# OllieBoyne/FIND

Hardware: AMD Instinct MI355X
Metric: deformed vertices x rendered views / sec (fwd+bwd) (higher is better)
Workload: dtype f32; 1 GPU; train_3d.yaml network-stage step: 16 feet x 6890-vertex template per GPU, 10002-vertex GT scans, chamf(5000)+smooth+texture(1000) losses, backward, Adam(main_params) step; nothing rendered, views:=1; feet_per_gpu=16, template_verts=6890, parallelism=dp1

## Files before the change

### find_amd/_lib.py

```python
import ctypes
import os
from ctypes import POINTER, Structure, c_char_p, c_float, c_int, c_int16, c_int32, c_int64, c_void_p

_PKG = os.path.dirname(os.path.abspath(__file__))
LIB_PATH = os.path.join(_PKG, 'lib', 'libfind_hip.so')
MAX_LAYERS = 8
ABI_VERSION = 3

_lib = None


class MlpParams(Structure):
	_fields_ = [
		('width', c_int32), ('in_dim', c_int32), ('pe_size', c_int32), ('n_trunk', c_int32),
		('n_disp', c_int32), ('n_col', c_int32), ('lat_disp', c_int32), ('lat_col', c_int32),
		('B', c_void_p),
		('trunk_w', c_void_p * MAX_LAYERS), ('trunk_b', c_void_p * MAX_LAYERS),
		('disp_w', c_void_p * MAX_LAYERS), ('disp_b', c_void_p * MAX_LAYERS),
		('col_w', c_void_p * MAX_LAYERS), ('col_b', c_void_p * MAX_LAYERS),
		('avg_col', c_void_p),
		('precision', c_int32),
	]


# ... 57 lines not shown
	'find_normal_map_bwd': (c_int, [_P, _P, _P, _I, _I, _I, _I, c_int, _P, _P]),
	'find_normal_loss_ws_bytes': (c_int64, [_I]),
	'find_normal_loss_fwd': (c_int, [_P, _P, _P, _I, _P, _P, _I, _P]),
	'find_normal_loss_bwd': (c_int, [_P, _P, _P, _I, _P, _P, _P, _P]),
	'find_point_face_ws_bytes': (c_int64, [_I, _I]),
	'find_point_face_fwd': (c_int, [_P, _P, _P, _P, _I, _I, _I, _I, _I, _P, _P, _P, _P, _I, _P]),
	'find_point_face_bwd': (c_int, [_P, _P, _P, _I, _P, _P, _P, _I, _I, _I, _I, _P, _P, _P]),
	'find_depth_bwd': (c_int, [POINTER(RenderParams), _P, _P, _I, _P, _P, _I, _I, _I, _I, _P, _P, _P, _P]),
	'find_depth_loss_ws_bytes': (c_int64, [_I, _I]),
	'find_depth_loss_fwd': (c_int, [_P, _P, _P, _I, _I, c_int, c_float, c_float, _P, _P, _P, _I, _P]),
	'find_depth_loss_bwd': (c_int, [_P, _P, _P, _I, _I, c_int, c_float, c_float, _P, _P, _P, _P]),
	'find_uv_sample': (c_int, [_P, _I, _I, _I, _P, _I, _P, _I, _I, _P, _P, _I, _I, _P, _P]),
	'find_render_frags': (c_int, [POINTER(RenderParams), _I, _I, _I, _I, _P, _P, _P, _P]),
	'find_adam_step': (c_int, [_I, _P, _P, _P, _P, _P, c_float, c_float, c_float, c_float, c_float, _I, _P]),
	'find_adam_step_dev': (c_int, [_I, _P, _P, _P, _P, _P, c_float, c_float, c_float, c_float, c_float, _P, _P]),
	'find_sgd_step': (c_int, [_I, _P, _P, _P, _P, c_float, c_float, c_float, c_float, c_int, c_int, _P]),
	'find_register_fwd': (c_int, [_P, _I, _P, _P, _I, _I, _P, _P]),
	'find_register_bwd_ws_bytes': (c_int64, [_I, _I]),
	'find_register_bwd': (c_int, [_P, _I, _P, _P, _P, _I, _I, _P, _P, _P, _I, _P]),
	'find_pca_fwd': (c_int, [_P, _I, _I, _P, _I, _P, _P]),
	'find_pca_bwd_ws_bytes': (c_int64, [_I, _I, _I]),
	'find_pca_bwd': (c_int, [_P, _I, _I, _P, _I, _P, _P, _I, _P]),
	'find_sample_points_fwd': (c_int, [_P, _P, _I, _P, _P, _I, _I, _I, _I, _P, _P, _P, _P]),
	'find_sample_points_bwd': (c_int, [_P, _I, _P, _P, _P, _I, _I, _I, _I, _P, _P]),
	'find_face_areas': (c_int, [_P, _P, _I, _I, _I, _I, _P, _P]),
	'find_nn_fwd': (c_int, [_P, _P, _P, _P, _I, _I, _I, _P, _P, _P]),
	'find_nn_bwd': (c_int, [_P, _P, _P, _P, _P, _I, _I, _I, _P, _P, _P]),
	'find_sample_surface_ws_bytes': (c_int64, [_I, _I]),
	'find_sample_surface_fwd': (c_int, [_P, _P, _I, _P, _I, _I, _I, _I, _P, _P, _P, _P, _P, _P, _I, _P]),
	'find_sample_surface_again': (c_int, [_P, _P, _I, _P, _I, _I, _I, _I, _P, _P, _P, _P, _P, _P, _I, _P]),
	'find_chamfer_ws_bytes': (c_int64, [_I, _I, _I]),
	'find_chamfer_fwd': (c_int, [_P, _P, _P, _P, _I, _I, _I, _P, _P, _I, _P]),
	'find_chamfer_bwd': (c_int, [_P, _P, _P, _P, _I, _I, _I, _P, _P, _I, _P, _P, _P]),
	'find_masked_mse_fwd': (c_int, [_P, _P, _I, _P, _P]),
	'find_masked_mse_bwd': (c_int, [_P, _P, _I, _P, _P, _P]),
	'find_image_mse_ws_bytes': (c_int64, []),
	'find_image_mse_fwd': (c_int, [_P, _P, _P, _P, _I, _I, _P, _P, _I, _P]),
	'find_image_mse_bwd': (c_int, [_P, _P, _P, _P, _I, _I, _P, _P, _P, _P]),
	'find_image_metrics_ws_bytes': (c_int64, [_I, _I]),
	'find_image_metrics': (c_int, [_P, _P, _P, _P, _P, _P, _I, _I, _I, _P, _P, _I, _P]),
	'find_smooth_loss_fwd': (c_int, [_P, _P, _P, _P, _P, _P, _I, _I, _I, _I, c_float, c_float, _P, _P, _I, _P]),
	'find_smooth_loss_bwd': (c_int, [_P, _P, _P, _P, _P, _P, _I, _I, _I, _I, c_float, c_float, _P, _P, _I, _P, _P]),
	'find_smooth_ws_bytes': (c_int64, [_I, _I, _I]),
	'find_smooth_fwd': (c_int, [_P, _P, _P, _P, _P, _P, _I, _I, _I, _I, _P, _P, _P, _I, _P]),
	'find_smooth_bwd': (c_int, [_P, _P, _P, _P, _P, _P, _I, _I, _I, _I, _P, _P, _P, _I, _P, _P]),
	'find_render_ws_bytes': (c_int64, [POINTER(RenderParams), _I, _I, _I, _I]),
	'find_render_fwd': (c_int, [POINTER(RenderParams), _P, _P, _I, _P, _P, _P, _I, _I, _I, _I, _P, _P, _P, _P, _P, _I, _P]),
	'find_render_bwd': (c_int, [POINTER(RenderParams), _P, _P, _I, _P, _P, _P, _I, _I, _I, _I, _P, _P, _P, _P, _P, _P, _I, _P]),
	'find_render_flags': (c_int, [_P, _P, _P]),
	'find_render_features_ws_bytes': (c_int64, [POINTER(RenderParams), _I, _I, _I]),
	'find_render_features_fwd': (c_int, [POINTER(RenderParams), _P, _P, _I, _P, _P, _I, _I, _I, _I, _P, _I, _P, _P, _I, _P, _I, _P]),
	'find_render_features_bwd': (c_int, [POINTER(RenderParams), _P, _P, _I, _P, _P, _I, _I, _I, _I, _P, _I, _P, _P, _P, _P, _P, _I, _P, _I, _P]),
	'find_points_render': (c_int, [POINTER(PointsParams), _P, _P, _P, _P, _I, _I, _I, _P, _P, _P, _P, _P]),
	'find_frames_u8': (c_int, [_P, _I, _I, _I, _I, c_int, _P, _P]),
}


def lib():
	global _lib
	if _lib is not None:
		return _lib
	if not os.path.exists(LIB_PATH):
		raise RuntimeError(f'find_amd: HIP library not built: {LIB_PATH} is missing. Run `python -m find_amd.build` '
						   '(or __graft_entry__.build()). There is no CPU fallback.')
	import torch
	L = ctypes.CDLL(LIB_PATH)
# ... 95 lines not shown
```

### find_amd/csrc/common.h

```cpp
#pragma once
#include <hip/hip_runtime.h>
#include <stdarg.h>
#include <stdint.h>
#include <stdio.h>
#include <string.h>
#include <algorithm>

#include "find_hip.h"

namespace find {

void set_error(const char* fmt, ...);
extern int g_raster_ablate;

constexpr int MLP_SWITCHES = 16 | 32 | 128;
constexpr int RASTER_SWITCHES = 8 | 16 | 256 | 512 | 1024 | 2048 | 4096 | 8192 | 16384 | 32768;

inline int check_launch(const char* what) {
	hipError_t e = hipGetLastError();
	if (e != hipSuccess) {
		set_error("%s: %s", what, hipGetErrorString(e));
		return FIND_ELAUNCH;
	}
	return FIND_OK;
}

inline int64_t align_up(int64_t x, int64_t a) { return (x + a - 1) / a * a; }
inline int64_t cdiv(int64_t a, int64_t b) { return (a + b - 1) / b; }

struct Carver {
	char* base;
	int64_t off;
	explicit Carver(void* p) : base(reinterpret_cast<char*>(p)), off(0) {}
	template <typename T>
	T* take(int64_t n) {
		T* r = reinterpret_cast<T*>(base + off);
		off += align_up(n * (int64_t)sizeof(T), 256);
		return r;
	}
};

}

#define FIND_REQUIRE(cond, ...)            \
	do {                                   \
		if (!(cond)) {                     \
			find::set_error(__VA_ARGS__);  \
			return FIND_EINVAL;            \
		}                                  \
// ... 26 lines not shown
```

### find_amd/csrc/geom.hip

```cpp
#include "common.h"

namespace find {
namespace geom {

__device__ __forceinline__ float3 ld3(const float* p) { return make_float3(p[0], p[1], p[2]); }
__device__ __forceinline__ float3 sub3(float3 a, float3 b) { return make_float3(a.x - b.x, a.y - b.y, a.z - b.z); }
__device__ __forceinline__ float3 cross3(float3 a, float3 b) {
	return make_float3(a.y * b.z - a.z * b.y, a.z * b.x - a.x * b.z, a.x * b.y - a.y * b.x);
}
__device__ __forceinline__ float norm3(float3 a) { return sqrtf(a.x * a.x + a.y * a.y + a.z * a.z); }

__global__ void face_areas_kernel(const float* __restrict__ verts, const int32_t* __restrict__ faces, int64_t faces_mesh_stride,
								  int n_verts, int n_faces, float* __restrict__ areas) {
	const int m = blockIdx.y;
	const int f = blockIdx.x * blockDim.x + threadIdx.x;
	if (f >= n_faces) return;
	const int32_t* fp = faces + (int64_t)m * faces_mesh_stride + (int64_t)f * 3;
	const float* vp = verts + (int64_t)m * n_verts * 3;
	if (fp[0] < 0) {
		areas[(int64_t)m * n_faces + f] = 0.f;
		return;
	}
	const float3 a = ld3(vp + 3 * fp[0]), b = ld3(vp + 3 * fp[1]), c = ld3(vp + 3 * fp[2]);
	areas[(int64_t)m * n_faces + f] = 0.5f * norm3(cross3(sub3(b, a), sub3(c, a)));
// ... 479 lines not shown
		float total = 0.f;
		for (int i = 0; i < 2 * n_clouds; ++i) total += __builtin_nontemporal_load(partial + i);
		*loss = total / (float)max(n_clouds, 1);
	}
}

__global__ void chamfer_bwd_kernel(const float* __restrict__ x, const int32_t* __restrict__ x_len, int p1_max, const float* __restrict__ y,
								   const int32_t* __restrict__ y_len, int p2_max, const unsigned long long* __restrict__ kx,
								   const unsigned long long* __restrict__ ky, const float* __restrict__ g_loss, int n_clouds,
								   float* __restrict__ d_x, float* __restrict__ d_y) {
	const int n = blockIdx.y, dir = blockIdx.z;
	const int i = blockIdx.x * blockDim.x + threadIdx.x;
	const int pa_max = dir ? p2_max : p1_max, pb_max = dir ? p1_max : p2_max;
	const int32_t* la = dir ? y_len : x_len;
	const int pa = la ? la[n] : pa_max;
	if (i >= pa) return;
	const unsigned long long v = (dir ? ky : kx)[(int64_t)n * pa_max + i];
	if (v == ~0ull) return;
	const int j = (int)(unsigned)v;
	const float* ap = (dir ? y : x) + ((int64_t)n * pa_max + i) * 3;
	const float* bp = (dir ? x : y) + ((int64_t)n * pb_max + j) * 3;
	const float g = 2.0f * (*g_loss) / ((float)n_clouds * (float)max(pa, 1));
	const float gx = g * (ap[0] - bp[0]), gy = g * (ap[1] - bp[1]), gz = g * (ap[2] - bp[2]);
	float* da = dir ? d_y : d_x;
	float* db = dir ? d_x : d_y;
	if (da) {
		float* o = da + ((int64_t)n * pa_max + i) * 3;
		unsafeAtomicAdd(o + 0, gx); unsafeAtomicAdd(o + 1, gy); unsafeAtomicAdd(o + 2, gz);
	}
	if (db) {
		float* o = db + ((int64_t)n * pb_max + j) * 3;
		unsafeAtomicAdd(o + 0, -gx); unsafeAtomicAdd(o + 1, -gy); unsafeAtomicAdd(o + 2, -gz);
	}
}

__global__ void nn_bwd_kernel(const float* __restrict__ x, const int32_t* __restrict__ x_len, const float* __restrict__ y,
							  const int32_t* __restrict__ idx, const float* __restrict__ w, int p1_max, int p2_max,
							  float* __restrict__ d_x, float* __restrict__ d_y) {
	const int n = blockIdx.y;
	const int i = blockIdx.x * blockDim.x + threadIdx.x;
	const int p1 = x_len ? x_len[n] : p1_max;
	if (i >= p1) return;
	const int64_t o = (int64_t)n * p1_max + i;
	const int j = idx[o];
	if (j < 0) return;
	const float g = 2.0f * w[o];
	const float* xp = x + o * 3;
	const float* yp = y + ((int64_t)n * p2_max + j) * 3;
	const float gx = g * (xp[0] - yp[0]), gy = g * (xp[1] - yp[1]), gz = g * (xp[2] - yp[2]);
	if (d_x) {
		d_x[o * 3 + 0] += gx; d_x[o * 3 + 1] += gy; d_x[o * 3 + 2] += gz;
	}
	if (d_y) {
		float* dy = d_y + ((int64_t)n * p2_max + j) * 3;
		atomicAdd(dy + 0, -gx); atomicAdd(dy + 1, -gy); atomicAdd(dy + 2, -gz);
	}
}

__global__ void cot_weights_kernel(const float* __restrict__ verts, const int32_t* __restrict__ faces, int n_verts, int n_faces,
								   float* __restrict__ fw) {
#pragma clang fp contract(off)
	const int m = blockIdx.y;
	const int f = blockIdx.x * blockDim.x + threadIdx.x;
	if (f >= n_faces) return;
	const int32_t* fp = faces + (int64_t)f * 3;
	const float* vp = verts + (int64_t)m * n_verts * 3;
// ... 823 lines not shown
	a.d[0] = NnDir{x, x_len, y, y_len, (int)p1_max, (int)p2_max, nullptr, nullptr, w.kx};
	a.d[1] = NnDir{y, y_len, x, x_len, (int)p2_max, (int)p1_max, nullptr, nullptr, w.ky};
	a.n_dirs = 2;
	a.counter = w.counter;
	const int64_t p_max = std::max(p1_max, p2_max);
	int np;
	nn_shape(cdiv(p_max, 128) * n * 2, std::min(p1_max, p2_max), &np, &a.splits);
	if (a.splits > 1) {
		hipError_t e = hipMemsetAsync(ws, 0xff, (size_t)w.key_bytes, s);
		if (e != hipSuccess) { set_error("find_chamfer_fwd: hipMemsetAsync: %s", hipGetErrorString(e)); return FIND_ELAUNCH; }
	}
	int rc = launch_nn(a, np, p_max, n, s);
	if (rc != FIND_OK) return rc;
	hipLaunchKernelGGL(chamfer_reduce_kernel, dim3((unsigned)n, 2), dim3(1024), 0, s, w.kx, x_len, (int)p1_max, w.ky, y_len, (int)p2_max, (int)n, w.partial, w.counter,
					   loss);
	FIND_LAUNCH_CHECK("chamfer_reduce_kernel");
	return FIND_OK;
}

extern "C" int find_chamfer_bwd(const float* x, const int32_t* x_len, const float* y, const int32_t* y_len, int64_t n, int64_t p1_max, int64_t p2_max,
								const float* g_loss, const void* ws, int64_t ws_bytes, float* d_x, float* d_y, void* stream) {
	FIND_REQUIRE(x && y && g_loss && ws, "find_chamfer_bwd: NULL argument");
	FIND_REQUIRE(d_x || d_y, "find_chamfer_bwd: both gradient outputs NULL");
	FIND_REQUIRE(!bad_dims(n, p1_max) && !bad_dims(n, p2_max), "find_chamfer_bwd: bad sizes");
	ChamferWs w;
	carve_chamfer(n, p1_max, p2_max, const_cast<void*>(ws), &w);
	if (ws_bytes < w.bytes) { set_error("find_chamfer_bwd: workspace too small"); return FIND_EWORKSPACE; }
	hipLaunchKernelGGL(chamfer_bwd_kernel, dim3((unsigned)cdiv(std::max(p1_max, p2_max), 256), (unsigned)n, 2), dim3(256), 0, (hipStream_t)stream, x, x_len,
					   (int)p1_max, y, y_len, (int)p2_max, w.kx, w.ky, g_loss, (int)n, d_x, d_y);
	FIND_LAUNCH_CHECK("chamfer_bwd_kernel");
	return FIND_OK;
}

extern "C" int64_t find_sample_surface_ws_bytes(int64_t n_meshes, int64_t n_faces) {
	if (bad_dims(n_meshes, n_faces)) return -1;
	return align_up(n_meshes * n_faces * (int64_t)sizeof(float), 256);
}

extern "C" int find_sample_surface_fwd(const float* verts, const int32_t* faces, int64_t faces_batch, const float* rnd, int64_t n_meshes, int64_t n_verts,
									   int64_t n_faces, int64_t n_samples, int32_t* face_idx, float* uv, float* out, const float* attr, float* attr_out,
									   void* ws, int64_t ws_bytes, void* stream) {
	FIND_REQUIRE(verts && faces && rnd && face_idx && uv && out && ws, "find_sample_surface_fwd: NULL argument");
	FIND_REQUIRE((attr == nullptr) == (attr_out == nullptr), "find_sample_surface_fwd: attr and attr_out must both be given or both NULL");
	FIND_REQUIRE(!bad_dims(n_meshes, n_samples) && !bad_dims(n_meshes, n_faces) && n_verts >= 1, "find_sample_surface_fwd: bad sizes");
	FIND_REQUIRE(faces_batch == 1 || faces_batch == n_meshes, "find_sample_surface_fwd: faces_batch must be 1 or n_meshes");
	if (ws_bytes < find_sample_surface_ws_bytes(n_meshes, n_faces)) { set_error("find_sample_surface_fwd: workspace too small"); return FIND_EWORKSPACE; }
	hipStream_t s = (hipStream_t)stream;
	const int64_t fstride = faces_batch == 1 ? 0 : n_faces * 3;
	hipLaunchKernelGGL(face_areas_kernel, dim3((unsigned)cdiv(n_faces, 256), (unsigned)n_meshes), dim3(256), 0, s, verts, faces, fstride, (int)n_verts, (int)n_faces,
					   (float*)ws);
	hipLaunchKernelGGL(area_scan_kernel, dim3((unsigned)n_meshes), dim3(1024), 0, s, (int)n_faces, (float*)ws);
	hipLaunchKernelGGL(sample_surface_kernel, dim3((unsigned)cdiv(n_samples, 256), (unsigned)n_meshes), dim3(256), 0, s, verts, faces, fstride, (const float*)ws, rnd,
					   (int)n_verts, (int)n_faces, (int)n_samples, face_idx, uv, out, attr, attr_out);
	FIND_LAUNCH_CHECK("sample_surface");
	return FIND_OK;
}

extern "C" int find_sample_surface_again(const float* verts, const int32_t* faces, int64_t faces_batch, const float* rnd, int64_t n_meshes, int64_t n_verts,
										 int64_t n_faces, int64_t n_samples, int32_t* face_idx, float* uv, float* out, const float* attr, float* attr_out,
										 const void* ws, int64_t ws_bytes, void* stream) {
	FIND_REQUIRE(verts && faces && rnd && face_idx && uv && out && ws, "find_sample_surface_again: NULL argument");
	FIND_REQUIRE((attr == nullptr) == (attr_out == nullptr), "find_sample_surface_again: attr and attr_out must both be given or both NULL");
	FIND_REQUIRE(!bad_dims(n_meshes, n_samples) && !bad_dims(n_meshes, n_faces) && n_verts >= 1, "find_sample_surface_again: bad sizes");
	FIND_REQUIRE(faces_batch == 1 || faces_batch == n_meshes, "find_sample_surface_again: faces_batch must be 1 or n_meshes");
	if (ws_bytes < find_sample_surface_ws_bytes(n_meshes, n_faces)) { set_error("find_sample_surface_again: workspace too small"); return FIND_EWORKSPACE; }
	const int64_t fstride = faces_batch == 1 ? 0 : n_faces * 3;
// ... 131 lines not shown
```

### find_amd/functional.py

```python
import ctypes

import torch

from . import _lib
from ._lib import MlpGrads, MlpParams, check, current_stream, ptr


def _require_gpu(*tensors):
	for t in tensors:
		if t is None:
			continue
		if not t.is_cuda:
			raise RuntimeError('find_amd: the HIP path needs tensors on a ROCm device (got a CPU tensor); '
							   'there is no CPU fallback -- use oracle/ only for testing')
		if t.dtype != torch.float32 and t.is_floating_point():
			raise RuntimeError(f'find_amd: fp32 tensors required, got {t.dtype}')


def _c(t):
	return None if t is None else t.contiguous()


def _ws(nbytes, device):
	return torch.empty(max(int(nbytes), 256), dtype=torch.uint8, device=device)
# ... 613 lines not shown
		F = faces.shape[-2]
		out = torch.empty(N, S, 3, device=verts.device, dtype=torch.float32)
		aout = torch.empty_like(out) if attr is not None else None
		check(L.find_sample_points_fwd(ptr(verts), ptr(faces), fb, ptr(face_idx), ptr(uv), N, V, F, S, ptr(out), ptr(attr), ptr(aout),
									   current_stream(verts.device)), 'find_sample_points_fwd')
		ctx.save_for_backward(faces, face_idx, uv)
		ctx.dims = (N, V, F, S, fb)
		ctx.has_attr = attr is not None
		ctx.set_materialize_grads(False)
		if attr is None:
			return out
		return out, aout

	@staticmethod
	def backward(ctx, g_out, g_attr=None):
		L = _lib.lib()
		faces, face_idx, uv = ctx.saved_tensors
		N, V, F, S, fb = ctx.dims

		def scatter(g):
			if g is None:
				return None
			d = torch.zeros(N, V, 3, device=g.device, dtype=torch.float32)
			check(L.find_sample_points_bwd(ptr(faces), fb, ptr(face_idx), ptr(uv), ptr(_c(g)), N, V, F, S, ptr(d), current_stream(g.device)),
				  'find_sample_points_bwd')
			return d

		d_verts = scatter(g_out) if ctx.needs_input_grad[0] else None
		d_attr = scatter(g_attr) if (ctx.has_attr and ctx.needs_input_grad[4]) else None
		return d_verts, None, None, None, d_attr


def sample_points(verts, faces, face_idx, uv, attr=None):
	return _SamplePoints.apply(verts, faces, face_idx, uv, attr)


class _NoCtx:
	needs_input_grad = (False,) * 64

	def save_for_backward(self, *tensors):
		pass

	def mark_non_differentiable(self, *tensors):
		pass

	def set_materialize_grads(self, value):
		pass


_NO_CTX = _NoCtx()
CACHE_AREA_SUMS = _os.environ.get('FIND_CACHE_AREA_SUMS', '1') != '0'
_AREA_SUMS = {}
_AREA_SUM_OWNERS = {}


class _SampleSurface(torch.autograd.Function):

	@staticmethod
	def forward(ctx, verts, faces, rnd, attr):
		_require_gpu(verts, rnd, attr)
		L = _lib.lib()
		verts_in, faces_in = verts, faces
		verts, rnd, attr = _c(verts), _c(rnd), _c(attr)
		faces = _faces_i32(faces)
		N, V, _ = verts.shape
		S = rnd.shape[1]
		if rnd.shape != (N, S, 3):
# ... 32 lines not shown
					del _AREA_SUM_OWNERS[k]
		ctx.save_for_backward(faces, face_idx, uv)
		ctx.dims = (N, V, F, S, fb)
		ctx.has_attr = attr is not None
		ctx.mark_non_differentiable(face_idx, uv)
		ctx.set_materialize_grads(False)
		if attr is None:
			return out, face_idx, uv
		return out, aout, face_idx, uv

	@staticmethod
	def backward(ctx, g_out, *rest):
		L = _lib.lib()
		faces, face_idx, uv = ctx.saved_tensors
		N, V, F, S, fb = ctx.dims
		g_attr = rest[0] if ctx.has_attr else None

		def scatter(g):
			if g is None:
				return None
			d = torch.zeros(N, V, 3, device=g.device, dtype=torch.float32)
			check(L.find_sample_points_bwd(ptr(faces), fb, ptr(face_idx), ptr(uv), ptr(_c(g)), N, V, F, S, ptr(d), current_stream(g.device)),
				  'find_sample_points_bwd')
			return d

		d_verts = scatter(g_out) if ctx.needs_input_grad[0] else None
		d_attr = scatter(g_attr) if (ctx.has_attr and ctx.needs_input_grad[3]) else None
		return d_verts, None, None, d_attr


def sample_surface(verts, faces, rnd, attr=None):
	if torch.is_grad_enabled() and (verts.requires_grad or (attr is not None and attr.requires_grad)):
		r = _SampleSurface.apply(verts, faces, rnd, attr)
	else:
		r = _SampleSurface.forward(_NO_CTX, verts, faces, rnd, attr)
	if attr is None:
		return r[0], None, r[1], r[2]
	return r


class _PointFace(torch.autograd.Function):

	@staticmethod
	def forward(ctx, points, verts, faces, p_len):
		_require_gpu(points, verts)
		L = _lib.lib()
		points, verts = _c(points), _c(verts)
		faces = _faces_i32(faces)
		if points.dim() != 3 or verts.dim() != 3 or points.shape[-1] != 3 or verts.shape[-1] != 3 or verts.shape[0] != points.shape[0]:
			raise RuntimeError(f'find_amd.point_face_distance: points (N, P, 3) and verts (N, V, 3) expected, got {tuple(points.shape)} / {tuple(verts.shape)}')
		N, P, _ = points.shape
		V = verts.shape[1]
		if faces.dim() not in (2, 3) or faces.shape[-1] != 3 or (faces.dim() == 3 and faces.shape[0] not in (1, N)):
			raise RuntimeError(f'find_amd.point_face_distance: faces (F, 3) or ({N}, F, 3) expected, got {tuple(faces.shape)}')
		fb = 1 if faces.dim() == 2 else faces.shape[0]
		F = faces.shape[-2]
		dev = points.device
		pl = None if p_len is None else torch.as_tensor(p_len).to(device=dev, dtype=torch.int32).contiguous()
		dist2 = torch.empty(N, P, device=dev, dtype=torch.float32)
		idx = torch.empty(N, P, device=dev, dtype=torch.int32)
		bary = torch.empty(N, P, 3, device=dev, dtype=torch.float32)
		ws = _ws(L.find_point_face_ws_bytes(N, P), dev)
		check(L.find_point_face_fwd(ptr(points), ptr(pl), ptr(verts), ptr(faces), fb, N, P, V, F, ptr(dist2), ptr(idx), ptr(bary), ptr(ws), ws.numel(),
									current_stream(dev)), 'find_point_face_fwd')
		ctx.save_for_backward(points, verts, faces, idx, bary)
		ctx.dims = (N, P, V, F, fb)
# ... 70 lines not shown
		P2 = y.shape[1]
		if y.shape[0] != N:
			raise RuntimeError('find_amd.chamfer_distance: batch mismatch')
		dev = x.device
		xl = None if x_len is None else x_len.to(device=dev, dtype=torch.int32).contiguous()
		yl = None if y_len is None else y_len.to(device=dev, dtype=torch.int32).contiguous()
		ws = _ws(L.find_chamfer_ws_bytes(N, P1, P2), dev)
		loss = torch.empty((), device=dev, dtype=torch.float32)
		check(L.find_chamfer_fwd(ptr(x), ptr(xl), ptr(y), ptr(yl), N, P1, P2, ptr(loss), ptr(ws), ws.numel(), current_stream(dev)), 'find_chamfer_fwd')
		ctx.save_for_backward(x, y, ws)
		ctx.lens = (xl, yl)
		return loss

	@staticmethod
	def backward(ctx, g):
		L = _lib.lib()
		x, y, ws = ctx.saved_tensors
		xl, yl = ctx.lens
		N, P1, _ = x.shape
		P2 = y.shape[1]
		need_x, need_y = ctx.needs_input_grad[0], ctx.needs_input_grad[1]
		if not (need_x or need_y):
			return None, None, None, None
		buf = torch.zeros((N * P1 * 3 if need_x else 0) + (N * P2 * 3 if need_y else 0), device=x.device, dtype=torch.float32)
		d_x = buf[:N * P1 * 3].view(N, P1, 3) if need_x else None
		d_y = buf[buf.numel() - N * P2 * 3:].view(N, P2, 3) if need_y else None
		check(L.find_chamfer_bwd(ptr(x), ptr(xl), ptr(y), ptr(yl), N, P1, P2, ptr(_c(g)), ptr(ws), ws.numel(), ptr(d_x), ptr(d_y), current_stream(x.device)),
			  'find_chamfer_bwd')
		return d_x, d_y, None, None


def chamfer_distance(x, y, x_lengths=None, y_lengths=None):
	return _Chamfer.apply(x, y, x_lengths, y_lengths), None


class _MaskedMSE(torch.autograd.Function):
	@staticmethod
	def forward(ctx, pred, target):
		_require_gpu(pred, target)
		L = _lib.lib()
		pred, target = _c(pred), _c(target.detach())
		if pred.shape != target.shape or pred.shape[-1] != 3:
			raise RuntimeError(f'find_amd.masked_mse: pred {tuple(pred.shape)} and target {tuple(target.shape)} must both be (..., 3)')
		loss = torch.empty((), device=pred.device, dtype=torch.float32)
		check(L.find_masked_mse_fwd(ptr(pred), ptr(target), pred.numel() // 3, ptr(loss), current_stream(pred.device)), 'find_masked_mse_fwd')
		ctx.save_for_backward(pred, target)
		return loss

	@staticmethod
	def backward(ctx, g):
		L = _lib.lib()
		pred, target = ctx.saved_tensors
		d = torch.empty_like(pred)
		check(L.find_masked_mse_bwd(ptr(pred), ptr(target), pred.numel() // 3, ptr(_c(g)), ptr(d), current_stream(pred.device)), 'find_masked_mse_bwd')
		return d, None


def masked_mse(pred, target):
	return _MaskedMSE.apply(pred, target)


class _ImageMSE(torch.autograd.Function):

	@staticmethod
	def forward(ctx, a, am, b, bm):
		_require_gpu(a, am, b, bm)
# ... 439 lines not shown
```

### find_amd/losses.py

```python
import itertools

import numpy as np
import torch

from . import functional as FN
from . import functional_render as FR
from .structures import Meshes, TexturesUV, TexturesVertex

nn = torch.nn


def sample_points_from_meshes(meshes: Meshes, num_samples: int = 10000, return_textures: bool = False, generator=None, draws=None):
	verts = meshes.verts_padded()
	faces = meshes.faces_shared()
	if faces is None:
		faces = meshes.faces_padded()
	N = verts.shape[0]
	tex = meshes.textures if return_textures else None
	if return_textures and not isinstance(tex, (TexturesUV, TexturesVertex)):
		raise NotImplementedError('return_textures needs TexturesVertex or TexturesUV')
	attr = tex.verts_features_padded()[..., :3].contiguous() if isinstance(tex, TexturesVertex) else None
	if draws is None:
		rnd = torch.rand(N, num_samples, 3, device=verts.device, generator=generator)
		pts, cols, face_idx, uv = FN.sample_surface(verts, faces, rnd, attr)
	else:
		face_idx, uv = draws
		r = FN.sample_points(verts, faces, face_idx, uv, attr)
		pts, cols = r if attr is not None else (r, None)
	if not return_textures:
		return pts
	if isinstance(tex, TexturesUV):
		su = uv[..., 0].sqrt()
		bary = torch.stack([1.0 - su, su * (1.0 - uv[..., 1]), su * uv[..., 1]], dim=-1)
		return pts, FR.uv_sample(tex.maps_padded(), tex.verts_uvs_padded(), tex.faces_uvs_padded(), face_idx, bary)
	return pts, cols


def _compact_by_mask(points, keep):
	order = torch.argsort((~keep).to(torch.int8), dim=1, stable=True)
	return torch.gather(points, 1, order.unsqueeze(-1).expand(-1, -1, 3)), keep.sum(dim=1).to(torch.int32)


def chamfer_distance(x, y, x_lengths=None, y_lengths=None):
	return FN.chamfer_distance(x, y, x_lengths, y_lengths)


def _mesh_faces(meshes):
	faces = meshes.faces_shared()
	return faces if faces is not None else meshes.faces_padded()


def point_mesh_distance(points, meshes: Meshes, lengths=None):
	return FN.point_face_distance(points, meshes.verts_padded(), _mesh_faces(meshes), lengths)


class TextureLossGTSpace(nn.Module):
	def forward(self, model, batch: dict, num_samples=1000, shapevec=None, texvec=None, posevec=None, gt_samples=None) -> torch.Tensor:
		mesh_gt = batch['mesh']
		sampled_verts, sampled_gt_colours = gt_samples if gt_samples is not None else sample_points_from_meshes(mesh_gt, num_samples=num_samples, return_textures=True)
		texvec = texvec if texvec is not None else batch.get('texvec', None)
		shapevec = shapevec if shapevec is not None else batch.get('shapevec', None)
		posevec = posevec if posevec is not None else batch.get('posevec', None)
		only_col = dict(want=('col',), defer_wgrad_join=True) if 'want' in getattr(getattr(model.forward, '__code__', None), 'co_varnames', ()) else {}
		res = model(sampled_verts.detach(), texvec=texvec, shapevec=shapevec, posevec=posevec, **only_col)
		return FN.masked_mse(res['col'], sampled_gt_colours)


class DisplacementLoss(nn.Module):
	def forward(self, model, res, batch, epoch, num_samples=5000, z_cutoff=None, gt_z_cutoff=None, gt_samples=None):
		if gt_samples is None:
			gt_samples = sample_points_from_meshes(batch['mesh'], num_samples=num_samples)
		pred_samples = sample_points_from_meshes(res['meshes'], num_samples=num_samples)
		if z_cutoff is not None:
			p, pl = _compact_by_mask(pred_samples, pred_samples[..., 2] <= z_cutoff)
			g, gl = _compact_by_mask(gt_samples, gt_samples[..., 2] <= z_cutoff)
			chamf_loss, _ = chamfer_distance(p, g, pl, gl)
		elif gt_z_cutoff is not None:
			g, gl = _compact_by_mask(gt_samples, gt_samples[..., 2] <= gt_z_cutoff)
			chamf_loss, _ = chamfer_distance(pred_samples, g, None, gl)
		else:
			chamf_loss, _ = chamfer_distance(pred_samples, gt_samples)
		return dict(loss=chamf_loss)


class MeshSmoothnessLoss(nn.Module):
	def forward(self, meshes: Meshes):
		faces = meshes.faces_shared()
		if faces is None:
			raise NotImplementedError('MeshSmoothnessLoss expects meshes sharing one topology (the template), as on the FIND path')
		verts = meshes.verts_padded()
		topo = FN.MeshTopology.get(faces, verts.shape[1])
		return FN.mesh_smoothness_loss(verts, topo, w_edge=10.0, w_lap=0.1)


class SilhouetteLoss(nn.Module):
	def forward(self, pred, gt):
		return FN.image_mse(pred, gt)


def draw_pairs(N, npairs=10):
	max_pairs = (N * (N - 1)) // 2
	npairs = min(npairs, max_pairs)
	all_pairs = list(itertools.permutations(np.arange(N), 2))
	np.random.shuffle(all_pairs)
	return np.array(all_pairs[:npairs], dtype=np.int32).reshape(-1, 2)
# ... 92 lines not shown
```

### include/find_hip.h

```cpp
#ifndef FIND_HIP_H
#define FIND_HIP_H

#include <stdint.h>

#ifdef __cplusplus
extern "C" {
#endif

#define FIND_ABI_VERSION 3

#define FIND_OK 0
#define FIND_EINVAL (-1)
#define FIND_EWORKSPACE (-2)
#define FIND_ELAUNCH (-3)

#define FIND_MAX_LAYERS 8

int find_abi_version(void);
const char* find_last_error(void);
const char* find_build_arch(void);

typedef struct find_ctx find_ctx;
int find_ctx_create(int device, find_ctx** out);
int find_ctx_destroy(find_ctx* ctx);
// ... 104 lines not shown
					  const float* d_out, int64_t n_feet, int64_t n_pts, float* d_disp, float* d_reg,
					  void* ws, int64_t ws_bytes, void* stream);

int find_pca_fwd(const float* coefs, int64_t V, int64_t B, const float* shapevec, int64_t n_feet, float* offsets, void* stream);
int64_t find_pca_bwd_ws_bytes(int64_t n_feet, int64_t V, int64_t B);
int find_pca_bwd(const float* coefs, int64_t V, int64_t B, const float* d_offsets, int64_t n_feet, float* d_shapevec, void* ws, int64_t ws_bytes,
				 void* stream);

int find_sample_points_fwd(const float* verts, const int32_t* faces, int64_t faces_batch, const int32_t* face_idx,
						   const float* uv, int64_t n_meshes, int64_t n_verts, int64_t n_faces, int64_t n_samples,
						   float* out, const float* attr, float* attr_out, void* stream);
int find_sample_points_bwd(const int32_t* faces, int64_t faces_batch, const int32_t* face_idx, const float* uv,
						   const float* d_out, int64_t n_meshes, int64_t n_verts, int64_t n_faces, int64_t n_samples,
						   float* d_verts, void* stream);
int find_face_areas(const float* verts, const int32_t* faces, int64_t faces_batch, int64_t n_meshes, int64_t n_verts,
					int64_t n_faces, float* areas, void* stream);
int64_t find_sample_surface_ws_bytes(int64_t n_meshes, int64_t n_faces);
int find_sample_surface_fwd(const float* verts, const int32_t* faces, int64_t faces_batch, const float* rnd, int64_t n_meshes,
							int64_t n_verts, int64_t n_faces, int64_t n_samples, int32_t* face_idx, float* uv, float* out,
							const float* attr, float* attr_out, void* ws, int64_t ws_bytes, void* stream);
int find_sample_surface_again(const float* verts, const int32_t* faces, int64_t faces_batch, const float* rnd, int64_t n_meshes,
							  int64_t n_verts, int64_t n_faces, int64_t n_samples, int32_t* face_idx, float* uv, float* out,
							  const float* attr, float* attr_out, const void* ws, int64_t ws_bytes, void* stream);

int find_nn_fwd(const float* x, const int32_t* x_len, const float* y, const int32_t* y_len, int64_t n,
				int64_t p1_max, int64_t p2_max, float* dist, int32_t* idx, void* stream);
int find_nn_bwd(const float* x, const int32_t* x_len, const float* y, const int32_t* idx, const float* w, int64_t n,
				int64_t p1_max, int64_t p2_max, float* d_x, float* d_y, void* stream);
int64_t find_chamfer_ws_bytes(int64_t n, int64_t p1_max, int64_t p2_max);
int find_chamfer_fwd(const float* x, const int32_t* x_len, const float* y, const int32_t* y_len, int64_t n, int64_t p1_max,
					 int64_t p2_max, float* loss, void* ws, int64_t ws_bytes, void* stream);
int find_chamfer_bwd(const float* x, const int32_t* x_len, const float* y, const int32_t* y_len, int64_t n, int64_t p1_max,
					 int64_t p2_max, const float* g_loss, const void* ws, int64_t ws_bytes, float* d_x, float* d_y, void* stream);

int find_masked_mse_fwd(const float* pred, const float* target, int64_t n_pts, float* loss, void* stream);
int find_masked_mse_bwd(const float* pred, const float* target, int64_t n_pts, const float* g_loss, float* d_pred, void* stream);
int64_t find_image_mse_ws_bytes(void);
int find_image_mse_fwd(const float* a, const float* a_mask, const float* b, const float* b_mask, int64_t n_pix, int64_t channels, float* loss,
					   void* ws, int64_t ws_bytes, void* stream);
int find_image_mse_bwd(const float* a, const float* a_mask, const float* b, const float* b_mask, int64_t n_pix, int64_t channels,
					   const float* g_loss, float* d_a, float* d_a_mask, void* stream);

#define FIND_IMAGE_METRIC_SQ 0
#define FIND_IMAGE_METRIC_SQ_EACH 1
#define FIND_IMAGE_METRIC_SQ_COMMON 2
#define FIND_IMAGE_METRIC_INTER 3
#define FIND_IMAGE_METRIC_UNION 4
#define FIND_IMAGE_METRIC_WSQ 5
#define FIND_IMAGE_METRIC_W 6
#define FIND_IMAGE_METRIC_COUNT 7
int64_t find_image_metrics_ws_bytes(int64_t n_img, int64_t n_pix);
int find_image_metrics(const float* pred, const float* gt, const float* pred_mask, const float* gt_mask, const uint8_t* hide, const float* weight,
					   int64_t n_img, int64_t n_pix, int64_t channels, double* sums, void* ws, int64_t ws_bytes, void* stream);

int64_t find_smooth_ws_bytes(int64_t n_meshes, int64_t n_verts, int64_t n_faces);
int find_smooth_fwd(const float* verts, const int32_t* faces, const int32_t* vf_off, const int32_t* vf_items,
					const int32_t* nbr_off, const int32_t* nbr_idx, int64_t n_meshes, int64_t n_verts, int64_t n_faces,
					int64_t n_edges, float* loss_edge, float* loss_lap, void* ws, int64_t ws_bytes, void* stream);
int find_smooth_bwd(const float* verts, const int32_t* faces, const int32_t* vf_off, const int32_t* vf_items,
					const int32_t* nbr_off, const int32_t* nbr_idx, int64_t n_meshes, int64_t n_verts, int64_t n_faces,
					int64_t n_edges, const float* g_edge, const float* g_lap, void* ws, int64_t ws_bytes, float* d_verts,
					void* stream);
int find_smooth_loss_fwd(const float* verts, const int32_t* faces, const int32_t* vf_off, const int32_t* vf_items,
						 const int32_t* nbr_off, const int32_t* nbr_idx, int64_t n_meshes, int64_t n_verts, int64_t n_faces,
						 int64_t n_edges, float w_edge, float w_lap, float* loss, void* ws, int64_t ws_bytes, void* stream);
int find_smooth_loss_bwd(const float* verts, const int32_t* faces, const int32_t* vf_off, const int32_t* vf_items,
// ... 81 lines not shown
```

Measured before the change: 73.17 million vertices*views/s.

## Fuse chamfer backward with surface-sample scatter into vertex gradients in LDS

Adds a fused backward kernel that computes chamfer gradients for the sampled points and scatters them through barycentric weights straight into a per-workgroup LDS image of vertex gradients. It replaces the separate chamfer backward, the sample-points backward and their global atomics. Large batches are split into slices whose partial results go to a workspace and are summed by a second kernel. The Python loss path uses it by default when the shapes fit in LDS, which adds LDS CAS loops and a dependence on sample metadata attached to tensors.

Result: faster. 74.97 million vertices*views/s, median of 6 (+2.5%).

```diff
diff --git a/find_amd/_lib.py b/find_amd/_lib.py
--- a/find_amd/_lib.py
+++ b/find_amd/_lib.py
@@ -113,6 +113,8 @@
 	'find_chamfer_ws_bytes': (c_int64, [_I, _I, _I]),
 	'find_chamfer_fwd': (c_int, [_P, _P, _P, _P, _I, _I, _I, _P, _P, _I, _P]),
 	'find_chamfer_bwd': (c_int, [_P, _P, _P, _P, _I, _I, _I, _P, _P, _I, _P, _P, _P]),
+	'find_chamfer_surface_bwd_ws_bytes': (c_int64, [_I, _I, _I]),
+	'find_chamfer_surface_bwd': (c_int, [_P, _P, _P, _I, _I, _I, _P, _P, _I, _P, _I, _P, _P, _I, _I, _P, _P, _I, _P]),
 	'find_masked_mse_fwd': (c_int, [_P, _P, _I, _P, _P]),
 	'find_masked_mse_bwd': (c_int, [_P, _P, _I, _P, _P, _P]),
 	'find_image_mse_ws_bytes': (c_int64, []),
diff --git a/find_amd/csrc/common.h b/find_amd/csrc/common.h
--- a/find_amd/csrc/common.h
+++ b/find_amd/csrc/common.h
@@ -14,7 +14,7 @@
 extern int g_raster_ablate;
 
 constexpr int MLP_SWITCHES = 16 | 32 | 128;
-constexpr int RASTER_SWITCHES = 8 | 16 | 256 | 512 | 1024 | 2048 | 4096 | 8192 | 16384 | 32768;
+constexpr int RASTER_SWITCHES = 8 | 16 | 256 | 512 | 1024 | 2048 | 4096 | 8192 | 16384 | 32768 | 0x70000;
 
 inline int check_launch(const char* what) {
 	hipError_t e = hipGetLastError();
diff --git a/find_amd/csrc/geom.hip b/find_amd/csrc/geom.hip
--- a/find_amd/csrc/geom.hip
+++ b/find_amd/csrc/geom.hip
@@ -535,6 +535,197 @@
 		float* o = db + ((int64_t)n * pb_max + j) * 3;
 		unsafeAtomicAdd(o + 0, -gx); unsafeAtomicAdd(o + 1, -gy); unsafeAtomicAdd(o + 2, -gz);
 	}
+}
+
+constexpr int SCB_THREADS = 1024, SCB_BATCH = 5;
+constexpr int64_t SCB_LDS_MAX = 160 * 1024;
+struct SurfBwdArgs {
+	const float *x, *y;
+	const int32_t* y_len;
+	const unsigned long long *kx, *ky;
+	const float* g_loss;
+	const int32_t* faces;
+	int64_t faces_mesh_stride;
+	const int32_t* face_idx;
+	const float* uv;
+	int p1, p2_max, n_clouds, n_verts, n_faces;
+	int range;
+	float* out;
+	int64_t out_foot_stride, out_slice_stride;
+};
+
+template <int N>
+__device__ __forceinline__ void lds_add_cas(unsigned* const (&word)[N], const float (&add)[N], unsigned (&cur)[N], bool (&open)[N]) {
+	bool any = true;
+	while (any) {
+		unsigned got[N];
+#pragma unroll
+		for (int k = 0; k < N; ++k)
+			if (open[k]) got[k] = atomicCAS(word[k], cur[k], __float_as_uint(__uint_as_float(cur[k]) + add[k]));
+		any = false;
+#pragma unroll
+		for (int k = 0; k < N; ++k)
+			if (open[k]) {
+				open[k] = got[k] != cur[k];
+				cur[k] = got[k];
+				any = any || open[k];
+			}
+	}
+}
+
+__global__ __launch_bounds__(SCB_THREADS) void chamfer_surface_bwd_kernel(const SurfBwdArgs a) {
+	extern __shared__ __attribute__((aligned(16))) float scb_lds[];
+	const int tid = threadIdx.x, n = blockIdx.y, slice = blockIdx.x;
+	const int V3 = a.n_verts * 3;
+	float* dst = a.out + (int64_t)n * a.out_foot_stride + (int64_t)slice * a.out_slice_stride;
+	const int head = (int)((reinterpret_cast<uintptr_t>(dst) >> 2) & 3);
+	float* img = scb_lds + head;
+	const int n_quads = (head + V3 + 3) >> 2;
+	float* dxs = scb_lds + ((V3 + 3 + 3) & ~3);
+	for (int q = tid; q < n_quads; q += SCB_THREADS) reinterpret_cast<float4*>(scb_lds)[q] = make_float4(0.f, 0.f, 0.f, 0.f);
+
+	const int p1 = a.p1, p2_max = a.p2_max;
+	const int p2_len = a.y_len ? a.y_len[n] : p2_max;
+	const int p2 = min(max(p2_len, 0), p2_max);
+	const float gl = *a.g_loss;
+	const float c0 = 2.0f * gl / ((float)a.n_clouds * (float)max(p1, 1));
+	const float c1 = 2.0f * gl / ((float)a.n_clouds * (float)max(p2_len, 1));
+	const int r0 = min((int)((int64_t)slice * a.range), p1), r1 = min(r0 + a.range, p1);
+	const float* xn = a.x + (int64_t)n * p1 * 3;
+	const float* yn = a.y + (int64_t)n * p2_max * 3;
+	const unsigned long long* kxn = a.kx + (int64_t)n * p1;
+	const unsigned long long* kyn = a.ky + (int64_t)n * p2_max;
+	const int32_t* fin = a.face_idx + (int64_t)n * p1;
+	const float* uvn = a.uv + (int64_t)n * p1 * 2;
+	const int32_t* fn = a.faces + (int64_t)n * a.faces_mesh_stride;
+
+	for (int s0 = r0; s0 < r1; s0 += SCB_THREADS * SCB_BATCH) {
+		unsigned long long key[SCB_BATCH];
+		int s[SCB_BATCH];
+#pragma unroll
+		for (int b = 0; b < SCB_BATCH; ++b) {
+			s[b] = s0 + b * SCB_THREADS + tid;
+			key[b] = kxn[min(s[b], r1 - 1)];
+		}
+		float3 pa[SCB_BATCH], pb[SCB_BATCH];
+		bool ok[SCB_BATCH];
+#pragma unroll
+		for (int b = 0; b < SCB_BATCH; ++b) {
+			const unsigned j = (unsigned)key[b];
+			ok[b] = key[b] != ~0ull && j < (unsigned)p2_max;
+			pa[b] = ld3(xn + (int64_t)min(s[b], r1 - 1) * 3);
+			pb[b] = ld3(yn + (int64_t)(ok[b] ? j : 0u) * 3);
+		}
+#pragma unroll
+		for (int b = 0; b < SCB_BATCH; ++b) {
+			if (s[b] >= r1) continue;
+			float* o = dxs + (s[b] - r0) * 3;
+			o[0] = ok[b] ? c0 * (pa[b].x - pb[b].x) : 0.f;
+			o[1] = ok[b] ? c0 * (pa[b].y - pb[b].y) : 0.f;
+			o[2] = ok[b] ? c0 * (pa[b].z - pb[b].z) : 0.f;
+		}
+	}
+	__syncthreads();
+
+	for (int k0 = 0; k0 < p2; k0 += SCB_THREADS * SCB_BATCH) {
+		unsigned long long key[SCB_BATCH];
+		int k[SCB_BATCH];
+#pragma unroll
+		for (int b = 0; b < SCB_BATCH; ++b) {
+			k[b] = k0 + b * SCB_THREADS + tid;
+			key[b] = kyn[min(k[b], p2 - 1)];
+		}
+		float3 pa[SCB_BATCH], pb[SCB_BATCH];
+		bool ok[SCB_BATCH];
+		int j[SCB_BATCH];
+#pragma unroll
+		for (int b = 0; b < SCB_BATCH; ++b) {
+			j[b] = (int)(unsigned)key[b];
+			ok[b] = k[b] < p2 && key[b] != ~0ull && j[b] >= r0 && j[b] < r1;
+			j[b] = ok[b] ? j[b] : r0;
+			pa[b] = ld3(yn + (int64_t)min(k[b], p2 - 1) * 3);
+			pb[b] = ld3(xn + (int64_t)min(j[b], p1 - 1) * 3);
+		}
+#pragma unroll
+		for (int b = 0; b < SCB_BATCH; ++b) {
+			if (!ok[b]) continue;
+			unsigned* row = reinterpret_cast<unsigned*>(dxs) + (j[b] - r0) * 3;
+			unsigned* const word[3] = {row, row + 1, row + 2};
+			const float add[3] = {-c1 * (pa[b].x - pb[b].x), -c1 * (pa[b].y - pb[b].y), -c1 * (pa[b].z - pb[b].z)};
+			typedef volatile __attribute__((address_space(3))) unsigned lds_word;
+			unsigned cur[3] = {*(lds_word*)row, *(lds_word*)(row + 1), *(lds_word*)(row + 2)};
+			bool open[3] = {true, true, true};
+			lds_add_cas<3>(word, add, cur, open);
+		}
+	}
+	__syncthreads();
+
+	for (int s0 = r0; s0 < r1; s0 += SCB_THREADS * SCB_BATCH) {
+		int s[SCB_BATCH], face[SCB_BATCH];
+		float u[SCB_BATCH][2];
+#pragma unroll
+		for (int b = 0; b < SCB_BATCH; ++b) {
+			s[b] = s0 + b * SCB_THREADS + tid;
+			const int ss = min(s[b], r1 - 1);
+			face[b] = fin[ss];
+			u[b][0] = uvn[(int64_t)ss * 2 + 0];
+			u[b][1] = uvn[(int64_t)ss * 2 + 1];
+		}
+		int vi[SCB_BATCH][3];
+		bool ok[SCB_BATCH];
+#pragma unroll
+		for (int b = 0; b < SCB_BATCH; ++b) {
+			ok[b] = s[b] < r1 && (unsigned)face[b] < (unsigned)a.n_faces;
+			const int32_t* fp = fn + (int64_t)(ok[b] ? face[b] : 0) * 3;
+			vi[b][0] = fp[0]; vi[b][1] = fp[1]; vi[b][2] = fp[2];
+		}
+#pragma unroll
+		for (int b = 0; b < SCB_BATCH; ++b) {
+			if (!ok[b]) continue;
+			const float* d = dxs + (s[b] - r0) * 3;
+			const float gx = d[0], gy = d[1], gz = d[2];
+			float w[3];
+			bary_weights(u[b], w);
+			unsigned* word[9];
+			float add[9];
+			unsigned cur[9];
+			bool open[9];
+#pragma unroll
+			for (int c = 0; c < 3; ++c) {
+				const bool in = (unsigned)vi[b][c] < (unsigned)a.n_verts;
+				unsigned* row = reinterpret_cast<unsigned*>(img) + 3 * (in ? vi[b][c] : 0);
+				word[3 * c + 0] = row + 0; word[3 * c + 1] = row + 1; word[3 * c + 2] = row + 2;
+				add[3 * c + 0] = w[c] * gx; add[3 * c + 1] = w[c] * gy; add[3 * c + 2] = w[c] * gz;
+				open[3 * c + 0] = open[3 * c + 1] = open[3 * c + 2] = in;
+				cur[3 * c + 0] = cur[3 * c + 1] = cur[3 * c + 2] = 0u;
+			}
+			lds_add_cas<9>(word, add, cur, open);
+		}
+	}
+	__syncthreads();
+
+	for (int q = tid; q < n_quads; q += SCB_THREADS) {
+		const float4 v = reinterpret_cast<const float4*>(scb_lds)[q];
+		const int e = 4 * q - head;
+		if (e >= 0 && e + 3 < V3) {
+			*reinterpret_cast<float4*>(dst + e) = v;
+		} else {
+			const float r[4] = {v.x, v.y, v.z, v.w};
+#pragma unroll
+			for (int k = 0; k < 4; ++k)
+				if (e + k >= 0 && e + k < V3) dst[e + k] = r[k];
+		}
+	}
+}
+
+__global__ __launch_bounds__(256) void chamfer_surface_sum_kernel(const float* __restrict__ slabs, int n_slices, int64_t slab_stride, int V3,
+																  float* __restrict__ d_verts) {
+	const int n = blockIdx.y, e = blockIdx.x * 256 + threadIdx.x;
+	if (e >= V3) return;
+	const float* p = slabs + (int64_t)n * n_slices * slab_stride + e;
+	float s = 0.f;
+	for (int k = 0; k < n_slices; ++k) s += p[(int64_t)k * slab_stride];
+	d_verts[(int64_t)n * V3 + e] = s;
 }
 
 __global__ void nn_bwd_kernel(const float* __restrict__ x, const int32_t* __restrict__ x_len, const float* __restrict__ y,
@@ -1424,6 +1615,61 @@
 	return FIND_OK;
 }
 
+static int surf_bwd_slices(int64_t n, int64_t n_samples) {
+	const int forced = (g_raster_ablate >> 16) & 7;
+	if (forced) return 1 << (forced - 1);
+	if (n_samples <= SCB_THREADS) return 1;
+	return n <= 16 ? 8 : n <= 32 ? 4 : n <= 128 ? 2 : 1;
+}
+static int64_t surf_bwd_lds(int64_t n_verts, int64_t range) { return align_up((((n_verts * 3 + 6) & ~(int64_t)3) + range * 3) * (int64_t)sizeof(float), 16); }
+
+extern "C" int64_t find_chamfer_surface_bwd_ws_bytes(int64_t n, int64_t n_verts, int64_t n_samples) {
+	if (bad_dims(n, n_samples) || n_verts < 1) return -1;
+	const int slices = surf_bwd_slices(n, n_samples);
+	if (surf_bwd_lds(n_verts, cdiv(n_samples, slices)) > SCB_LDS_MAX) return -1;
+	return slices == 1 ? 0 : n * slices * align_up(n_verts * 3, 64) * (int64_t)sizeof(float);
+}
+
+extern "C" int find_chamfer_surface_bwd(const float* x, const float* y, const int32_t* y_len, int64_t n, int64_t p1, int64_t p2_max, const float* g_loss,
+										const void* chamfer_ws, int64_t chamfer_ws_bytes, const int32_t* faces, int64_t faces_batch, const int32_t* face_idx,
+										const float* uv, int64_t n_verts, int64_t n_faces, float* d_verts, void* ws, int64_t ws_bytes, void* stream) {
+	FIND_REQUIRE(x && y && g_loss && chamfer_ws && faces && face_idx && uv && d_verts, "find_chamfer_surface_bwd: NULL argument");
+	FIND_REQUIRE(!bad_dims(n, p1) && !bad_dims(n, p2_max) && n_verts >= 1 && !bad_dims(n, n_faces), "find_chamfer_surface_bwd: bad sizes");
+	FIND_REQUIRE(faces_batch == 1 || faces_batch == n, "find_chamfer_surface_bwd: faces_batch must be 1 or n");
+	const int64_t need = find_chamfer_surface_bwd_ws_bytes(n, n_verts, p1);
+	FIND_REQUIRE(need >= 0, "find_chamfer_surface_bwd: %lld vertices do not fit one workgroup's LDS (find_chamfer_surface_bwd_ws_bytes < 0)", (long long)n_verts);
+	ChamferWs w;
+	carve_chamfer(n, p1, p2_max, const_cast<void*>(chamfer_ws), &w);
+	if (chamfer_ws_bytes < w.bytes) { set_error("find_chamfer_surface_bwd: Chamfer workspace too small"); return FIND_EWORKSPACE; }
+	if (ws_bytes < need || (need > 0 && !ws)) { set_error("find_chamfer_surface_bwd: workspace too small"); return FIND_EWORKSPACE; }
+	const int slices = surf_bwd_slices(n, p1);
+	const int64_t slab = align_up(n_verts * 3, 64);
+	const int lds = (int)surf_bwd_lds(n_verts, cdiv(p1, slices));
+	static bool lds_granted[64] = {};
+	int dev = 0;
+	if (lds > 64 * 1024 && (hipGetDevice(&dev) != hipSuccess || dev < 0 || dev >= 64 || !lds_granted[dev])) {
+		hipError_t e = hipFuncSetAttribute(reinterpret_cast<const void*>(&chamfer_surface_bwd_kernel), hipFuncAttributeMaxDynamicSharedMemorySize, (int)SCB_LDS_MAX);
+		if (e != hipSuccess) { set_error("find_chamfer_surface_bwd: hipFuncSetAttribute(MaxDynamicSharedMemorySize): %s", hipGetErrorString(e)); return FIND_ELAUNCH; }
+		if (dev >= 0 && dev < 64) lds_granted[dev] = true;
+	}
+	hipStream_t s = (hipStream_t)stream;
+	SurfBwdArgs a = {};
+	a.x = x; a.y = y; a.y_len = y_len; a.kx = w.kx; a.ky = w.ky; a.g_loss = g_loss;
+	a.faces = faces; a.faces_mesh_stride = faces_batch == 1 ? 0 : n_faces * 3; a.face_idx = face_idx; a.uv = uv;
+	a.p1 = (int)p1; a.p2_max = (int)p2_max; a.n_clouds = (int)n; a.n_verts = (int)n_verts; a.n_faces = (int)n_faces;
+	a.range = (int)cdiv(p1, slices);
+	if (slices == 1) { a.out = d_verts; a.out_foot_stride = n_verts * 3; a.out_slice_stride = 0; }
+	else { a.out = (float*)ws; a.out_foot_stride = slices * slab; a.out_slice_stride = slab; }
+	hipLaunchKernelGGL(chamfer_surface_bwd_kernel, dim3((unsigned)slices, (unsigned)n), dim3(SCB_THREADS), (size_t)lds, s, a);
+	FIND_LAUNCH_CHECK("chamfer_surface_bwd_kernel");
+	if (slices > 1) {
+		hipLaunchKernelGGL(chamfer_surface_sum_kernel, dim3((unsigned)cdiv(n_verts * 3, 256), (unsigned)n), dim3(256), 0, s, (const float*)ws, slices, slab, (int)(n_verts * 3),
+						   d_verts);
+		FIND_LAUNCH_CHECK("chamfer_surface_sum_kernel");
+	}
+	return FIND_OK;
+}
+
 extern "C" int64_t find_sample_surface_ws_bytes(int64_t n_meshes, int64_t n_faces) {
 	if (bad_dims(n_meshes, n_faces)) return -1;
 	return align_up(n_meshes * n_faces * (int64_t)sizeof(float), 256);
diff --git a/find_amd/functional.py b/find_amd/functional.py
--- a/find_amd/functional.py
+++ b/find_amd/functional.py
@@ -669,7 +669,10 @@
 
 
 def sample_points(verts, faces, face_idx, uv, attr=None):
-	return _SamplePoints.apply(verts, faces, face_idx, uv, attr)
+	r = _SamplePoints.apply(verts, faces, face_idx, uv, attr)
+	if attr is None and torch.is_grad_enabled() and verts.requires_grad:
+		_remember_surface(r, verts, _faces_i32(faces), face_idx.to(torch.int32).contiguous(), _c(uv))
+	return r
 
 
 class _NoCtx:
@@ -768,6 +771,8 @@
 def sample_surface(verts, faces, rnd, attr=None):
 	if torch.is_grad_enabled() and (verts.requires_grad or (attr is not None and attr.requires_grad)):
 		r = _SampleSurface.apply(verts, faces, rnd, attr)
+		if attr is None and verts.requires_grad:
+			_remember_surface(r[0], verts, _faces_i32(faces), r[1], r[2])
 	else:
 		r = _SampleSurface.forward(_NO_CTX, verts, faces, rnd, attr)
 	if attr is None:
@@ -904,6 +909,79 @@
 
 def chamfer_distance(x, y, x_lengths=None, y_lengths=None):
 	return _Chamfer.apply(x, y, x_lengths, y_lengths), None
+
+
+class _SurfaceChamfer(torch.autograd.Function):
+
+	@staticmethod
+	def forward(ctx, verts, x, faces, face_idx, uv, y, y_len):
+		_require_gpu(x, y)
+		L = _lib.lib()
+		x, y = _c(x), _c(y)
+		N, S, _ = x.shape
+		if y.dim() != 3 or y.shape[0] != N or y.shape[2] != 3:
+			raise RuntimeError(f'find_amd.surface_chamfer: y must be ({N}, P2, 3), got {tuple(y.shape)}')
+		P2 = y.shape[1]
+		dev = x.device
+		yl = None if y_len is None else y_len.to(device=dev, dtype=torch.int32).contiguous()
+		ws = _ws(L.find_chamfer_ws_bytes(N, S, P2), dev)
+		loss = torch.empty((), device=dev, dtype=torch.float32)
+		check(L.find_chamfer_fwd(ptr(x), None, ptr(y), ptr(yl), N, S, P2, ptr(loss), ptr(ws), ws.numel(), current_stream(dev)), 'find_chamfer_fwd')
+		ctx.save_for_backward(x, y, ws, faces, face_idx, uv)
+		ctx.y_len = yl
+		ctx.dims = (N, verts.shape[1], faces.shape[-2], S, P2, 1 if faces.dim() == 2 else faces.shape[0])
+		return loss
+
+	@staticmethod
+	def backward(ctx, g):
+		if not ctx.needs_input_grad[0]:
+			return (None,) * 7
+		L = _lib.lib()
+		x, y, ws, faces, face_idx, uv = ctx.saved_tensors
+		N, V, F, S, P2, fb = ctx.dims
+		dev = x.device
+		d_verts = torch.empty(N, V, 3, device=dev, dtype=torch.float32)
+		bws = _ws(L.find_chamfer_surface_bwd_ws_bytes(N, V, S), dev)
+		check(L.find_chamfer_surface_bwd(ptr(x), ptr(y), ptr(ctx.y_len), N, S, P2, ptr(_c(g)), ptr(ws), ws.numel(), ptr(faces), fb, ptr(face_idx), ptr(uv), V, F,
+										 ptr(d_verts), ptr(bws), bws.numel(), current_stream(dev)), 'find_chamfer_surface_bwd')
+		return d_verts, None, None, None, None, None, None
+
+
+def _remember_surface(samples, verts, faces, face_idx, uv):
+	samples._find_surface = (verts, faces, face_idx, uv)
+
+
+def surface_of(samples):
+	return getattr(samples, '_find_surface', None)
+
+
+def surface_chamfer_fits(n_meshes, n_verts, n_samples):
+	return _lib.lib().find_chamfer_surface_bwd_ws_bytes(n_meshes, n_verts, n_samples) >= 0
+
+
+def surface_chamfer_pays(n_meshes, n_samples):
+	return n_meshes * n_samples >= 16384
+
+
+def surface_chamfer_distance(samples, y, y_len=None):
+	src = surface_of(samples)
+	if src is None:
+		raise RuntimeError('find_amd.surface_chamfer_distance: the samples are not the direct output of sample_surface / sample_points on a mesh that takes a gradient')
+	verts, faces, face_idx, uv = src
+	if not surface_chamfer_fits(verts.shape[0], verts.shape[1], samples.shape[1]):
+		raise RuntimeError(f'find_amd.surface_chamfer: {verts.shape[1]} vertices do not fit the fused backward (surface_chamfer_fits); '
+						   'use chamfer_distance')
+	return _SurfaceChamfer.apply(verts, samples.detach(), faces, face_idx, uv, y, y_len)
+
+
+def surface_chamfer(verts, faces, rnd, y, y_len=None):
+	if not surface_chamfer_fits(verts.shape[0], verts.shape[1], rnd.shape[1]):
+		raise RuntimeError(f'find_amd.surface_chamfer: {verts.shape[1]} vertices do not fit the fused backward (surface_chamfer_fits); '
+						   'use sample_surface + chamfer_distance')
+	samples = sample_surface(verts, faces, rnd)[0]
+	if surface_of(samples) is None:
+		raise RuntimeError('find_amd.surface_chamfer: verts must require a gradient (otherwise use sample_surface + chamfer_distance)')
+	return surface_chamfer_distance(samples, y, y_len), samples
 
 
 class _MaskedMSE(torch.autograd.Function):
diff --git a/find_amd/losses.py b/find_amd/losses.py
--- a/find_amd/losses.py
+++ b/find_amd/losses.py
@@ -1,4 +1,5 @@
 import itertools
+import os
 
 import numpy as np
 import torch
@@ -8,6 +9,7 @@
 from .structures import Meshes, TexturesUV, TexturesVertex
 
 nn = torch.nn
+FUSED_CHAMFER_BWD = int(os.environ.get('FIND_FUSED_CHAMFER_BWD', '1'))
 
 
 def sample_points_from_meshes(meshes: Meshes, num_samples: int = 10000, return_textures: bool = False, generator=None, draws=None):
@@ -71,6 +73,11 @@
 		if gt_samples is None:
 			gt_samples = sample_points_from_meshes(batch['mesh'], num_samples=num_samples)
 		pred_samples = sample_points_from_meshes(res['meshes'], num_samples=num_samples)
+		src = FN.surface_of(pred_samples) if FUSED_CHAMFER_BWD and z_cutoff is None and torch.is_grad_enabled() and not gt_samples.requires_grad else None
+		if (src is not None and (FUSED_CHAMFER_BWD >= 2 or FN.surface_chamfer_pays(pred_samples.shape[0], pred_samples.shape[1]))
+				and FN.surface_chamfer_fits(pred_samples.shape[0], src[0].shape[1], pred_samples.shape[1])):
+			g, gl = _compact_by_mask(gt_samples, gt_samples[..., 2] <= gt_z_cutoff) if gt_z_cutoff is not None else (gt_samples, None)
+			return dict(loss=FN.surface_chamfer_distance(pred_samples, g, gl))
 		if z_cutoff is not None:
 			p, pl = _compact_by_mask(pred_samples, pred_samples[..., 2] <= z_cutoff)
 			g, gl = _compact_by_mask(gt_samples, gt_samples[..., 2] <= z_cutoff)
diff --git a/include/find_hip.h b/include/find_hip.h
--- a/include/find_hip.h
+++ b/include/find_hip.h
@@ -160,6 +160,11 @@
 					 int64_t p2_max, float* loss, void* ws, int64_t ws_bytes, void* stream);
 int find_chamfer_bwd(const float* x, const int32_t* x_len, const float* y, const int32_t* y_len, int64_t n, int64_t p1_max,
 					 int64_t p2_max, const float* g_loss, const void* ws, int64_t ws_bytes, float* d_x, float* d_y, void* stream);
+int64_t find_chamfer_surface_bwd_ws_bytes(int64_t n, int64_t n_verts, int64_t n_samples);
+int find_chamfer_surface_bwd(const float* x, const float* y, const int32_t* y_len, int64_t n, int64_t p1, int64_t p2_max,
+							 const float* g_loss, const void* chamfer_ws, int64_t chamfer_ws_bytes, const int32_t* faces,
+							 int64_t faces_batch, const int32_t* face_idx, const float* uv, int64_t n_verts, int64_t n_faces,
+							 float* d_verts, void* ws, int64_t ws_bytes, void* stream);
 
 int find_masked_mse_fwd(const float* pred, const float* target, int64_t n_pts, float* loss, void* stream);
 int find_masked_mse_bwd(const float* pred, const float* target, int64_t n_pts, const float* g_loss, float* d_pred, void* stream);
```
